# irconde/SSL4POLYP

Hardware: AMD Instinct MI355X
Metric: training-step images/sec/node, ViT-B/16 224^2 (cls fine-tune) (higher is better)
Workload: dtype bf16; 1 GPU; ViT-B/16 classification fine-tune, bs=64/GPU, 224^2, AdamW, random init, finetune mode full (finetune.py:49-91); global_batch=64, parallelism=dp1, launch=eager, lr_schedule=constant

## Files before the change

### ssl4polyp_amd/csrc/pm_attention.hip

```cpp
#include "pm_common.h"
#include <type_traits>

namespace {

template <int DH> constexpr int kTileUnroll = DH == 32 ? 2 : 1;

template <int RB> __device__ __forceinline__ int swz(int row) {
  if constexpr (RB == 64) return (row >> 2) & 3;
  else if constexpr (RB == 128) return (((row >> 1) & 1) << 2) | ((row >> 2) & 3);
  else if constexpr (RB == 384) return row & 7;
  else return row & 15;
}

constexpr int row_bytes_of(int esize, int dh) { return dh == 80 ? (esize == 2 ? 256 : 384) : dh * esize; }
template <typename T, int DH> constexpr int row_bytes() { return row_bytes_of((int)sizeof(T), DH); }

template <typename T, int DH>
__device__ __forceinline__ void load_image(char* img, const T* __restrict__ src, long ld, int rows_valid,
                                           int rows_total, int tid, int nthreads) {
  constexpr int RB = row_bytes<T, DH>();
  constexpr int CPV = DH * sizeof(T) / 16;
  constexpr int CPF = ((DH + 31) / 32) * 32 * sizeof(T) / 16;
  constexpr int EPC = 16 / sizeof(T);
  for (int id = tid; id < rows_total * CPF; id += nthreads) {
    const int row = id / CPF, c = id % CPF;
    u32x4 v = {0u, 0u, 0u, 0u};
    if (row < rows_valid && c < CPV) v = *reinterpret_cast<const u32x4*>(src + (long)row * ld + c * EPC);
    *reinterpret_cast<u32x4*>(img + row * RB + 16 * (c ^ swz<RB>(row))) = v;
  }
}

template <typename T, int DH>
__device__ __forceinline__ Frag16 frag_rows(const char* img, int rb, int kk, int lane) {
  constexpr int RB = row_bytes<T, DH>();
  const int row = rb + (lane & 31);
  const int c = 2 * kk + (lane >> 5);
  Frag16 f;
  f.u = *reinterpret_cast<const u32x4*>(img + row * RB + 16 * (c ^ swz<RB>(row)));
  return f;
}

template <typename T>
__device__ __forceinline__ Frag16 frag_global(const T* __restrict__ rowptr, bool valid, int kk, int lane) {
  constexpr int EPC = 16 / sizeof(T);
  Frag16 f;
  f.u = (u32x4){0u, 0u, 0u, 0u};
  if (valid) f.u = *reinterpret_cast<const u32x4*>(rowptr + (2 * kk + (lane >> 5)) * EPC);
  return f;
}

template <typename T, int DH>
__device__ __forceinline__ f32x16 mma_imgT_acc(const char* PM_LDS_IMAGE img, int rb, int d0, const f32x16& x, f32x16 acc, int lane) {
  constexpr int RB = row_bytes<T, DH>();
  if constexpr (sizeof(T) == 2) {
    const int g = lane >> 4, i = lane & 15, q = i >> 2, p = i & 3, hh = g >> 1;
    const int col = d0 + 16 * (g & 1) + 4 * p;
    const int c = col >> 3, sub = 8 * (p & 1);
    using lds_s4 = __attribute__((address_space(3))) short4v;
#pragma unroll
    for (int s = 0; s < 2; ++s) {
      Frag16 a, b;
      const int r0 = rb + 16 * s + 4 * hh + q;
      const int r1 = r0 + 8;
      const short4v lo = __builtin_amdgcn_ds_read_tr16_b64_v4i16((lds_s4*)(img + r0 * RB + 16 * (c ^ swz<RB>(r0)) + sub));
      const short4v hi = __builtin_amdgcn_ds_read_tr16_b64_v4i16((lds_s4*)(img + r1 * RB + 16 * (c ^ swz<RB>(r1)) + sub));
      a.u[0] = ((unsigned)(unsigned short)lo[0]) | (((unsigned)(unsigned short)lo[1]) << 16);
      a.u[1] = ((unsigned)(unsigned short)lo[2]) | (((unsigned)(unsigned short)lo[3]) << 16);
      a.u[2] = ((unsigned)(unsigned short)hi[0]) | (((unsigned)(unsigned short)hi[1]) << 16);
      a.u[3] = ((unsigned)(unsigned short)hi[2]) | (((unsigned)(unsigned short)hi[3]) << 16);
#pragma unroll
      for (int j = 0; j < 8; ++j) frag_set<T>(b, j, x[8 * s + j]);
      acc = mfma16B<T>(a, b, acc);
    }
  } else {
    const int hh = lane >> 5;
    const int col = d0 + (lane & 31);
#pragma unroll
    for (int r = 0; r < 16; ++r) {
      const int row = rb + acc_row(r, hh);
      const float a = *reinterpret_cast<const float*>(img + row * RB + 16 * ((col >> 2) ^ swz<RB>(row)) + 4 * (col & 3));
      acc = __builtin_amdgcn_mfma_f32_32x32x2f32(a, x[r], acc, 0, 0, 0);
    }
  }
  return acc;
}

__device__ __forceinline__ f32x16 zero16() {
  f32x16 z;
#pragma unroll
  for (int r = 0; r < 16; ++r) z[r] = 0.f;
  return z;
}

template <typename T>
__device__ __forceinline__ void store_tile_T(T* __restrict__ rowptr, bool valid, const f32x16& acc, float scale, int lane,
                                             int ncols = 32) {
  if (!valid) return;
  const int hh = lane >> 5;
#pragma unroll
  for (int g = 0; g < 4; ++g) {
    f32x4 v = {acc[4 * g] * scale, acc[4 * g + 1] * scale, acc[4 * g + 2] * scale, acc[4 * g + 3] * scale};
    if (8 * g + 4 * hh < ncols) store4<T>(rowptr + 8 * g + 4 * hh, v);
  }
}
template <int DH> __device__ __forceinline__ constexpr int tile_cols(int dt) { return DH - 32 * dt < 32 ? DH - 32 * dt : 32; }

constexpr float kLog2e = 1.4426950408889634f;

template <int DH> __device__ __forceinline__ int problem_of_block(int bid, int nprob, int H) {
  if constexpr (DH == 32) {
    if ((nprob & 15) == 0 && (H & 1) == 0) {
      const int xcd = bid & 7, j = bid >> 3;
      return (((j >> 1) << 3) + xcd) * 2 + (j & 1);
    }
  }
  return bid;
}

constexpr int chunk_tiles(int row_bytes, int nt) {
  const int per_tile = 2 * 32 * row_bytes + 2 * 32 * (int)sizeof(float);
  if (nt * per_tile <= 150 * 1024) return nt;
  return (80 * 1024) / per_tile;
}

template <typename T, int DH, int NT, int CT>
__global__ __launch_bounds__(NT * 64) void attn_fwd_kernel(const T* __restrict__ qkv, T* __restrict__ out,
                                                                        float* __restrict__ lse, int N, int H,
                                                                        float scale) {
  constexpr int RB = row_bytes<T, DH>();
  constexpr int KS = DH * sizeof(T) / 32;
  constexpr int DT = (DH + 31) / 32;
  extern __shared__ __attribute__((aligned(16))) char smem[];
  char* imgK = smem;
  char* imgV = smem + CT * 32 * RB;
  const int tid = threadIdx.x, lane = tid & 63, wave = tid >> 6, hh = lane >> 5;
  const int prob = problem_of_block<DH>(blockIdx.x, gridDim.x, H);
  const int b = prob / H, h = prob % H;
  const long ld = 3L * H * DH;
  const T* base = qkv + (long)b * N * ld + h * DH;
  const float c = scale * kLog2e;
  const int q = wave * 32 + (lane & 31);
  const bool qv = q < N;
  Frag16 fq[KS];
  f32x16 o[DT];
#pragma unroll
  for (int dt = 0; dt < DT; ++dt) o[dt] = zero16();
  float m = -INFINITY, l = 0.f;
  for (int c0 = 0; c0 < NT; c0 += CT) {
    if (c0) __syncthreads();
    load_image<T, DH>(imgK, base + H * DH + (long)c0 * 32 * ld, ld, N - c0 * 32, CT * 32, tid, NT * 64);
    load_image<T, DH>(imgV, base + 2 * H * DH + (long)c0 * 32 * ld, ld, N - c0 * 32, CT * 32, tid, NT * 64);
    __syncthreads();
    if (c0 == 0) {
#pragma unroll
      for (int kk = 0; kk < KS; ++kk) fq[kk] = frag_global<T>(base + (long)q * ld, qv, kk, lane);
    }
    const int cend = c0 + CT < NT ? c0 + CT : NT;
#pragma unroll 1
    for (int kt = c0; kt < cend; ++kt) {
      const int rb = (kt - c0) * 32;
      f32x16 s = zero16();
#pragma unroll
      for (int kk = 0; kk < KS; ++kk) s = mfma16B<T>(frag_rows<T, DH>(imgK, rb, kk, lane), fq[kk], s);
      float tm = -INFINITY;
      if (kt * 32 + 32 > N) {
#pragma unroll
        for (int r = 0; r < 16; ++r) {
          const int key = kt * 32 + acc_row(r, hh);
          s[r] = key < N ? s[r] : -INFINITY;
        }
      }
#pragma unroll
      for (int r = 0; r < 16; ++r) tm = fmaxf(tm, s[r]);
      tm = fmaxf(tm, __shfl_xor(tm, 32, 64));
      const float mn = fmaxf(m, tm);
      const float alpha = __builtin_amdgcn_exp2f((m - mn) * c);
      const float mnc = mn * c;
      float ts = 0.f;
#pragma unroll
      for (int r = 0; r < 16; ++r) {
        s[r] = __builtin_amdgcn_exp2f(s[r] * c - mnc);
        ts += s[r];
      }
      l = l * alpha + ts;
      const bool moved = __builtin_amdgcn_ballot_w64(mn != m) != 0;
      m = mn;
#pragma unroll
      for (int dt = 0; dt < DT; ++dt) {
        if (moved) {
#pragma unroll
          for (int r = 0; r < 16; ++r) o[dt][r] *= alpha;
        }
        o[dt] = mma_imgT_acc<T, DH>(imgV, rb, dt * 32, s, o[dt], lane);
      }
    }
  }
  l += __shfl_xor(l, 32, 64);
  if (qv && hh == 0) lse[((long)b * H + h) * N + q] = m * scale + __logf(l);
  const float inv = 1.0f / l;
  T* orow = out + ((long)b * N + q) * H * DH + h * DH;
#pragma unroll
  for (int dt = 0; dt < DT; ++dt) store_tile_T<T>(orow + dt * 32, qv, o[dt], inv, lane, tile_cols<DH>(dt));
}

template <typename T, int DH, int NT, int CT>
__global__ __launch_bounds__(NT * 64) void attn_bwd_q_kernel(const T* __restrict__ qkv, const T* __restrict__ out,
                                                                          const T* __restrict__ dout,
                                                                          const float* __restrict__ lse,
                                                                          float* __restrict__ delta, T* __restrict__ dqkv,
                                                                          int N, int H, float scale) {
  constexpr int RB = row_bytes<T, DH>();
  constexpr int KS = DH * sizeof(T) / 32;
  constexpr int DT = (DH + 31) / 32;
  constexpr int EPC = 16 / sizeof(T);
  extern __shared__ __attribute__((aligned(16))) char smem[];
  char* imgK = smem;
  char* imgV = smem + CT * 32 * RB;
  const int tid = threadIdx.x, lane = tid & 63, wave = tid >> 6, hh = lane >> 5;
  const int prob = problem_of_block<DH>(blockIdx.x, gridDim.x, H);
  const int b = prob / H, h = prob % H;
  const long ld = 3L * H * DH, ldo = (long)H * DH;
  const T* base = qkv + (long)b * N * ld + h * DH;
  const float c = scale * kLog2e;
  const int q = wave * 32 + (lane & 31);
  const bool qv = q < N;
  const long sidx = ((long)b * H + h) * N + q;
  Frag16 fq[KS], fdo[KS];
  float l2 = 0.f, dls = 0.f;
  f32x16 dq[DT];
#pragma unroll
  for (int dt = 0; dt < DT; ++dt) dq[dt] = zero16();
  for (int c0 = 0; c0 < NT; c0 += CT) {
    if (c0) __syncthreads();
    load_image<T, DH>(imgK, base + H * DH + (long)c0 * 32 * ld, ld, N - c0 * 32, CT * 32, tid, NT * 64);
    load_image<T, DH>(imgV, base + 2 * H * DH + (long)c0 * 32 * ld, ld, N - c0 * 32, CT * 32, tid, NT * 64);
    __syncthreads();
    if (c0 == 0) {
      const T* orow = out + ((long)b * N + q) * ldo + h * DH;
      const T* dorow = dout + ((long)b * N + q) * ldo + h * DH;
      float dl = 0.f;
#pragma unroll
      for (int kk = 0; kk < KS; ++kk) {
        fq[kk] = frag_global<T>(base + (long)q * ld, qv, kk, lane);
        fdo[kk] = frag_global<T>(dorow, qv, kk, lane);
        const Frag16 fo = frag_global<T>(orow, qv, kk, lane);
#pragma unroll
        for (int e = 0; e < EPC; ++e) dl += frag_get<T>(fdo[kk], e) * frag_get<T>(fo, e);
      }
      dl += __shfl_xor(dl, 32, 64);
      if (qv && hh == 0) delta[sidx] = dl;
      l2 = qv ? lse[sidx] * kLog2e : 0.f;
      dls = dl * scale;
    }
    const int cend = c0 + CT < NT ? c0 + CT : NT;
#pragma unroll kTileUnroll<DH>
    for (int kt = c0; kt < cend; ++kt) {
      const int rb = (kt - c0) * 32;
      f32x16 s = zero16(), dp = zero16();
#pragma unroll
      for (int kk = 0; kk < KS; ++kk) {
        s = mfma16B<T>(frag_rows<T, DH>(imgK, rb, kk, lane), fq[kk], s);
        dp = mfma16B<T>(frag_rows<T, DH>(imgV, rb, kk, lane), fdo[kk], dp);
      }
#pragma unroll
      for (int r = 0; r < 16; ++r) s[r] = __builtin_amdgcn_exp2f(fminf(s[r] * c - l2, 0.f)) * (dp[r] * scale - dls);
#pragma unroll
      for (int dt = 0; dt < DT; ++dt) dq[dt] = mma_imgT_acc<T, DH>(imgK, rb, dt * 32, s, dq[dt], lane);
    }
  }
  T* dqrow = dqkv + ((long)b * N + q) * ld + h * DH;
#pragma unroll
  for (int dt = 0; dt < DT; ++dt) store_tile_T<T>(dqrow + dt * 32, qv, dq[dt], 1.0f, lane, tile_cols<DH>(dt));
}

template <typename T, int DH, int NT, int CT>
__global__ __launch_bounds__(NT * 64) void attn_bwd_kv_kernel(const T* __restrict__ qkv, const T* __restrict__ dout,
                                                                           const float* __restrict__ lse,
                                                                           const float* __restrict__ delta,
                                                                           T* __restrict__ dqkv, int N, int H, float scale) {
  constexpr int RB = row_bytes<T, DH>();
  constexpr int KS = DH * sizeof(T) / 32;
  constexpr int DT = (DH + 31) / 32;
  extern __shared__ __attribute__((aligned(16))) char smem[];
  char* imgQ = smem;
  char* imgDO = smem + CT * 32 * RB;
  float* sl2 = reinterpret_cast<float*>(smem + 2 * CT * 32 * RB);
  float* sdl = sl2 + CT * 32;
  const int tid = threadIdx.x, lane = tid & 63, wave = tid >> 6, hh = lane >> 5;
  const int prob = problem_of_block<DH>(blockIdx.x, gridDim.x, H);
  const int b = prob / H, h = prob % H;
  const long ld = 3L * H * DH, ldo = (long)H * DH;
  const T* base = qkv + (long)b * N * ld + h * DH;
  const float c = scale * kLog2e;
  const int key = wave * 32 + (lane & 31);
  const bool kv = key < N;
  Frag16 fk[KS], fv[KS];
  f32x16 dk[DT], dv[DT];
#pragma unroll
  for (int dt = 0; dt < DT; ++dt) {
    dk[dt] = zero16();
    dv[dt] = zero16();
  }
  for (int c0 = 0; c0 < NT; c0 += CT) {
    if (c0) __syncthreads();
    load_image<T, DH>(imgQ, base + (long)c0 * 32 * ld, ld, N - c0 * 32, CT * 32, tid, NT * 64);
    load_image<T, DH>(imgDO, dout + ((long)b * N + c0 * 32) * ldo + h * DH, ldo, N - c0 * 32, CT * 32, tid, NT * 64);
    for (int i = tid; i < CT * 32; i += NT * 64) {
      const int qi = c0 * 32 + i;
      const long sidx = ((long)b * H + h) * N + qi;
      sl2[i] = qi < N ? lse[sidx] * kLog2e : 0.f;
      sdl[i] = qi < N ? delta[sidx] * scale : 0.f;
    }
    __syncthreads();
    if (c0 == 0) {
#pragma unroll
      for (int kk = 0; kk < KS; ++kk) {
        fk[kk] = frag_global<T>(base + (long)key * ld + H * DH, kv, kk, lane);
        fv[kk] = frag_global<T>(base + (long)key * ld + 2 * H * DH, kv, kk, lane);
      }
    }
    const int cend = c0 + CT < NT ? c0 + CT : NT;
#pragma unroll kTileUnroll<DH>
    for (int qt = c0; qt < cend; ++qt) {
      const int rb = (qt - c0) * 32;
      f32x16 s = zero16(), dp = zero16();
#pragma unroll
      for (int kk = 0; kk < KS; ++kk) {
        s = mfma16B<T>(frag_rows<T, DH>(imgQ, rb, kk, lane), fk[kk], s);
        dp = mfma16B<T>(frag_rows<T, DH>(imgDO, rb, kk, lane), fv[kk], dp);
      }
#pragma unroll
      for (int g = 0; g < 4; ++g) {
        const int qq = rb + 8 * g + 4 * hh;
        const f32x4 l4 = *reinterpret_cast<const f32x4*>(sl2 + qq);
        const f32x4 d4 = *reinterpret_cast<const f32x4*>(sdl + qq);
#pragma unroll
        for (int e = 0; e < 4; ++e) {
          const int r = 4 * g + e;
          const float p = __builtin_amdgcn_exp2f(fminf(s[r] * c - l4[e], 0.f));
          s[r] = p;
          dp[r] = p * (dp[r] * scale - d4[e]);
        }
      }
#pragma unroll
      for (int dt = 0; dt < DT; ++dt) {
        dv[dt] = mma_imgT_acc<T, DH>(imgDO, rb, dt * 32, s, dv[dt], lane);
        dk[dt] = mma_imgT_acc<T, DH>(imgQ, rb, dt * 32, dp, dk[dt], lane);
      }
    }
  }
  T* drow = dqkv + ((long)b * N + key) * ld + h * DH;
#pragma unroll
  for (int dt = 0; dt < DT; ++dt) {
    store_tile_T<T>(drow + H * DH + dt * 32, kv, dk[dt], 1.0f, lane, tile_cols<DH>(dt));
    store_tile_T<T>(drow + 2 * H * DH + dt * 32, kv, dv[dt], 1.0f, lane, tile_cols<DH>(dt));
  }
}

template <int RB, typename T> __device__ __forceinline__ void dma_rows(char* img, const T* __restrict__ base, long ld, int rows_valid,
                                                                        int piece, int lane) {
  static_assert(sizeof(T) == 2, "16-bit rows");
  constexpr int CPR = RB / 16, RPP = 1024 / RB;
  const int row = piece * RPP + lane / CPR, cs = lane % CPR;
  const int c = cs ^ swz<RB>(row);
  const int gr = row < rows_valid ? row : rows_valid - 1;
  __builtin_amdgcn_global_load_lds((const __attribute__((address_space(1))) void*)(base + (long)gr * ld + c * 8),
                                   (__attribute__((address_space(3))) void*)(img + 1024 * piece), 16, 0, 0);
}

template <typename T, int DH, int NT>
__global__ __launch_bounds__(NT * 64) void attn_fwd2_kernel(const T* __restrict__ qkv, T* __restrict__ out,
                                                           float* __restrict__ lse, int N, int H, int BH, float scale) {
  constexpr int RB = DH * 2;
  constexpr int IMG = NT * 32 * RB;
  constexpr int PCS = IMG / 1024;
  constexpr int KS = RB / 32;
  constexpr int DT = DH / 32;
  extern __shared__ __attribute__((aligned(16))) char smem[];
  char* imgQ = smem + 4 * IMG;
  const int tid = threadIdx.x, lane = tid & 63, hh = lane >> 5;
  const int wave = __builtin_amdgcn_readfirstlane(tid >> 6);
  const long hd = (long)H * DH, ld = 3 * hd;
  const float c = scale * kLog2e;
  auto issue = [&](int head, int buf) {
    const int b = head / H, h = head % H;
    const T* base = qkv + (long)b * N * ld + (long)h * DH;
    char* imgK = smem + buf * 2 * IMG;
#pragma unroll
    for (int i = 0; i < (PCS + NT - 1) / NT; ++i) {
      const int p = wave + NT * i;
      if (p < PCS) {
        dma_rows<RB>(imgK, base + hd, ld, N, p, lane);
        dma_rows<RB>(imgK + IMG, base + 2 * hd, ld, N, p, lane);
        dma_rows<RB>(imgQ, base, ld, N, p, lane);
      }
    }
  };
  int head = blockIdx.x;
  if (head >= BH) return;
  issue(head, 0);
  for (int it = 0; head < BH; head += gridDim.x, ++it) {
    const int buf = it & 1;
    const char* imgK = smem + buf * 2 * IMG;
    const char* imgV = imgK + IMG;
    asm volatile("s_waitcnt vmcnt(0)" ::: "memory");
    __syncthreads();
    Frag16 fq[KS];
#pragma unroll
    for (int kk = 0; kk < KS; ++kk) fq[kk] = frag_rows<T, DH>(imgQ, wave * 32, kk, lane);
    asm volatile("s_waitcnt lgkmcnt(0)" ::: "memory");
    __builtin_amdgcn_sched_barrier(0);
    __syncthreads();
    const int next = head + gridDim.x;
    if (next < BH) issue(next, buf ^ 1);
    const int b = head / H, h = head % H;
    f32x16 s[NT];
#pragma unroll
    for (int kt = 0; kt < NT; ++kt) {
      s[kt] = zero16();
#pragma unroll
      for (int kk = 0; kk < KS; ++kk) s[kt] = mfma16B<T>(frag_rows<T, DH>(imgK, kt * 32, kk, lane), fq[kk], s[kt]);
    }
#pragma unroll
    for (int r = 0; r < 16; ++r) {
      const int key = (NT - 1) * 32 + acc_row(r, hh);
      s[NT - 1][r] = key < N ? s[NT - 1][r] : -INFINITY;
    }
    float m = -INFINITY;
#pragma unroll
    for (int kt = 0; kt < NT; ++kt)
#pragma unroll
      for (int r = 0; r < 16; r += 2) m = fmaxf(m, fmaxf(s[kt][r], s[kt][r + 1]));
    m = fmaxf(m, __shfl_xor(m, 32, 64));
    const float mc = m * c;
    f32x16 o[DT];
#pragma unroll
    for (int dt = 0; dt < DT; ++dt) o[dt] = zero16();
    float l = 0.f;
#pragma unroll
    for (int kt = 0; kt < NT; ++kt) {
#pragma unroll
      for (int r = 0; r < 16; ++r) {
        s[kt][r] = __builtin_amdgcn_exp2f(s[kt][r] * c - mc);
        l += s[kt][r];
      }
#pragma unroll
      for (int dt = 0; dt < DT; ++dt) o[dt] = mma_imgT_acc<T, DH>(imgV, kt * 32, dt * 32, s[kt], o[dt], lane);
    }
    l += __shfl_xor(l, 32, 64);
    const int q = wave * 32 + (lane & 31);
    const bool qv = q < N;
    if (qv && hh == 0) lse[((long)b * H + h) * N + q] = m * scale + __logf(l);
    const float inv = 1.0f / l;
    T* orow = out + ((long)b * N + q) * H * DH + h * DH;
#pragma unroll
    for (int dt = 0; dt < DT; ++dt) store_tile_T<T>(orow + dt * 32, qv, o[dt], inv, lane);
  }
}

template <typename T, int DH, int NT>
__global__ __launch_bounds__(NT * 64) void attn_bwd_fused_kernel(const T* __restrict__ qkv, const T* __restrict__ out,
                                                                const T* __restrict__ dout,
                                                                const float* __restrict__ lse, T* __restrict__ dqkv,
                                                                int N, int H, float scale) {
  constexpr int RB = DH * 2;
  constexpr int IMG = NT * 32 * RB;
  constexpr int PCS = IMG / 1024;
  constexpr int KS = RB / 32;
  constexpr int DT = DH / 32;
  constexpr int CPR = RB / 16;
  extern __shared__ __attribute__((aligned(16))) char smem[];
  char* imgQ = smem;
  char* imgK = smem + IMG;
  char* imgV = smem + 2 * IMG;
  char* imgDO = smem + 3 * IMG;
  float* sl2 = reinterpret_cast<float*>(smem + 4 * IMG);
  float* sdl = sl2 + NT * 32;
  const int tid = threadIdx.x, lane = tid & 63, hh = lane >> 5;
  const int wave = __builtin_amdgcn_readfirstlane(tid >> 6);
  const int prob = problem_of_block<DH>(blockIdx.x, gridDim.x, H);
  const int b = prob / H, h = prob % H;
  const long ld = 3L * H * DH, ldo = (long)H * DH;
  const T* base = qkv + (long)b * N * ld + h * DH;
  const T* dobase = dout + (long)b * N * ldo + h * DH;
#pragma unroll
  for (int i = 0; i < (PCS + NT - 1) / NT; ++i) {
    const int p = wave + NT * i;
    if (p < PCS) {
      dma_rows<RB>(imgQ, base, ld, N, p, lane);
      dma_rows<RB>(imgK, base + H * DH, ld, N, p, lane);
      dma_rows<RB>(imgV, base + 2 * H * DH, ld, N, p, lane);
      dma_rows<RB>(imgDO, dobase, ldo, N, p, lane);
    }
  }
  const int q = wave * 32 + (lane & 31);
  const bool qv = q < N;
  const long sidx = ((long)b * H + h) * N;
  Frag16 fo[KS];
  {
    const T* orow = out + ((long)b * N + (qv ? q : N - 1)) * ldo + h * DH;
#pragma unroll
    for (int kk = 0; kk < KS; ++kk) fo[kk].u = *reinterpret_cast<const u32x4*>(orow + (2 * kk + hh) * 8);
  }
  for (int i = tid; i < NT * 32; i += NT * 64) sl2[i] = i < N ? lse[sidx + i] * kLog2e : 0.f;
  asm volatile("s_waitcnt vmcnt(0)" ::: "memory");
  __syncthreads();
  {
    const int pad0 = N, npad = NT * 32 - N;
    for (int i = tid; i < npad * CPR; i += NT * 64) {
      const int off = (pad0 + i / CPR) * RB + 16 * (i % CPR);
      const u32x4 z = {0u, 0u, 0u, 0u};
      *reinterpret_cast<u32x4*>(imgQ + off) = z;
      *reinterpret_cast<u32x4*>(imgK + off) = z;
      *reinterpret_cast<u32x4*>(imgV + off) = z;
      *reinterpret_cast<u32x4*>(imgDO + off) = z;
    }
  }
  __syncthreads();
  const float c = scale * kLog2e;
  Frag16 fq[KS], fdo[KS];
  float dl = 0.f;
#pragma unroll
  for (int kk = 0; kk < KS; ++kk) {
    fq[kk] = frag_rows<T, DH>(imgQ, wave * 32, kk, lane);
    fdo[kk] = frag_rows<T, DH>(imgDO, wave * 32, kk, lane);
#pragma unroll
    for (int e = 0; e < 8; ++e) dl += frag_get<T>(fdo[kk], e) * frag_get<T>(fo[kk], e);
  }
  dl += __shfl_xor(dl, 32, 64);
  if (!qv) dl = 0.f;
  if (hh == 0) sdl[q] = dl * scale;
  {
    const float l2 = sl2[q];
    const float dls = dl * scale;
    f32x16 dq[DT];
#pragma unroll
    for (int dt = 0; dt < DT; ++dt) dq[dt] = zero16();
#pragma unroll kTileUnroll<DH>
    for (int kt = 0; kt < NT; ++kt) {
      f32x16 s = zero16(), dp = zero16();
#pragma unroll
      for (int kk = 0; kk < KS; ++kk) {
        s = mfma16B<T>(frag_rows<T, DH>(imgK, kt * 32, kk, lane), fq[kk], s);
        dp = mfma16B<T>(frag_rows<T, DH>(imgV, kt * 32, kk, lane), fdo[kk], dp);
      }
#pragma unroll
      for (int r = 0; r < 16; ++r) s[r] = __builtin_amdgcn_exp2f(fminf(s[r] * c - l2, 0.f)) * (dp[r] * scale - dls);
#pragma unroll
      for (int dt = 0; dt < DT; ++dt) dq[dt] = mma_imgT_acc<T, DH>(imgK, kt * 32, dt * 32, s, dq[dt], lane);
    }
    T* dqrow = dqkv + ((long)b * N + q) * ld + h * DH;
#pragma unroll
    for (int dt = 0; dt < DT; ++dt) store_tile_T<T>(dqrow + dt * 32, qv, dq[dt], 1.0f, lane);
  }
  __syncthreads();
  {
    const int key = q;
    const bool kv = qv;
    Frag16 fk[KS], fv[KS];
#pragma unroll
    for (int kk = 0; kk < KS; ++kk) {
      fk[kk] = frag_rows<T, DH>(imgK, wave * 32, kk, lane);
      fv[kk] = frag_rows<T, DH>(imgV, wave * 32, kk, lane);
    }
    f32x16 dk[DT], dv[DT];
#pragma unroll
    for (int dt = 0; dt < DT; ++dt) {
      dk[dt] = zero16();
      dv[dt] = zero16();
    }
#pragma unroll kTileUnroll<DH>
    for (int qt = 0; qt < NT; ++qt) {
      f32x16 s = zero16(), dp = zero16();
#pragma unroll
      for (int kk = 0; kk < KS; ++kk) {
        s = mfma16B<T>(frag_rows<T, DH>(imgQ, qt * 32, kk, lane), fk[kk], s);
        dp = mfma16B<T>(frag_rows<T, DH>(imgDO, qt * 32, kk, lane), fv[kk], dp);
      }
#pragma unroll
      for (int g = 0; g < 4; ++g) {
        const int qq = qt * 32 + 8 * g + 4 * hh;
        const f32x4 l4 = *reinterpret_cast<const f32x4*>(sl2 + qq);
        const f32x4 d4 = *reinterpret_cast<const f32x4*>(sdl + qq);
#pragma unroll
        for (int e = 0; e < 4; ++e) {
          const int r = 4 * g + e;
          const float pr = __builtin_amdgcn_exp2f(fminf(s[r] * c - l4[e], 0.f));
          s[r] = pr;
          dp[r] = pr * (dp[r] * scale - d4[e]);
        }
      }
#pragma unroll
      for (int dt = 0; dt < DT; ++dt) {
        dv[dt] = mma_imgT_acc<T, DH>(imgDO, qt * 32, dt * 32, s, dv[dt], lane);
        dk[dt] = mma_imgT_acc<T, DH>(imgQ, qt * 32, dt * 32, dp, dk[dt], lane);
      }
    }
    T* drow = dqkv + ((long)b * N + key) * ld + h * DH;
#pragma unroll
    for (int dt = 0; dt < DT; ++dt) {
      store_tile_T<T>(drow + H * DH + dt * 32, kv, dk[dt], 1.0f, lane);
      store_tile_T<T>(drow + 2 * H * DH + dt * 32, kv, dv[dt], 1.0f, lane);
    }
  }
}

int plan_attention(bool backward, int B, int N, int H, int dh, int dtype, pm_attention_plan_info* p) {
  if (B <= 0 || N <= 0 || H <= 0) return PM_ESHAPE;
  if (N > 288) return PM_ESHAPE;
  if (dh != 32 && dh != 64 && dh != 80) return PM_ESHAPE;
  if (dtype != PM_BF16 && dtype != PM_F16 && dtype != PM_F32) return PM_EINVAL;
  const int tiles = (N + 31) / 32, BH = B * H;
  const bool half = dtype != PM_F32;
  const int rb = row_bytes_of(half ? 2 : 4, dh);
  p->nt = dh == 80 ? (tiles <= 3 ? 3 : 9) : tiles <= 1 ? 1 : tiles <= 2 ? 2 : tiles <= 7 ? 7 : 9;
  p->ct = p->nt;
  p->grid = BH;
  p->launches = 1;
  p->lds_bytes[1] = 0;
  if (!backward && half && dh == 64 && tiles == 7) {
    p->family = PM_ATTN_FWD_PERSISTENT;
    const int rounds = (BH + 255) / 256;
    p->grid = (BH + rounds - 1) / rounds;
    p->lds_bytes[0] = 5 * 7 * 32 * dh * 2;
  } else if (!backward) {
    p->family = PM_ATTN_FWD_HEAD;
    p->ct = chunk_tiles(rb, p->nt);
    p->lds_bytes[0] = 2 * p->ct * 32 * rb;
  } else if (half && dh != 80) {
    p->family = PM_ATTN_BWD_FUSED;
    p->lds_bytes[0] = 4 * p->nt * 32 * rb + 2 * p->nt * 32 * sizeof(float);
  } else {
    p->family = PM_ATTN_BWD_SPLIT;
    p->launches = 2;
    p->ct = chunk_tiles(rb, p->nt);
    p->lds_bytes[0] = 2 * p->ct * 32 * rb;
    p->lds_bytes[1] = p->lds_bytes[0] + 2 * p->ct * 32 * sizeof(float);
  }
  return PM_OK;
}

template <int N> using Tiles = std::integral_constant<int, N>;
template <int DH, typename F> int with_nt(int nt, F&& f) {
  if constexpr (DH == 80) {
    if (nt == 3) return f(Tiles<3>{});
  } else {
    if (nt == 1) return f(Tiles<1>{});
    if (nt == 2) return f(Tiles<2>{});
    if (nt == 7) return f(Tiles<7>{});
  }
  return nt == 9 ? f(Tiles<9>{}) : PM_ESHAPE;
}

template <typename T, int DH>
int launch_fwd(const pm_attention_plan_info& p, const void* qkv, void* out, float* lse, int B, int N, int H, hipStream_t s) {
  const float scale = 1.0f / sqrtf((float)DH);
  if constexpr (sizeof(T) == 2 && DH == 64) {
    if (p.family == PM_ATTN_FWD_PERSISTENT) {
      auto kern = attn_fwd2_kernel<T, 64, 7>;
      PM_ALLOW_LDS(kern, p.lds_bytes[0]);
      hipLaunchKernelGGL(kern, dim3(p.grid), dim3(7 * 64), p.lds_bytes[0], s, (const T*)qkv, (T*)out, lse, N, H, B * H, scale);
      return pm_check_launch();
    }
  }
  return with_nt<DH>(p.nt, [&](auto nt) {
    constexpr int NT = decltype(nt)::value;
    auto kern = attn_fwd_kernel<T, DH, NT, chunk_tiles(row_bytes<T, DH>(), NT)>;
    PM_ALLOW_LDS(kern, p.lds_bytes[0]);
    hipLaunchKernelGGL(kern, dim3(p.grid), dim3(NT * 64), p.lds_bytes[0], s, (const T*)qkv, (T*)out, lse, N, H, scale);
    return pm_check_launch();
  });
}

template <typename T, int DH>
int launch_bwd(const pm_attention_plan_info& p, const void* qkv, const void* out, const void* dout, const float* lse, float* delta,
               void* dqkv, int B, int N, int H, hipStream_t s) {
  const float scale = 1.0f / sqrtf((float)DH);
  return with_nt<DH>(p.nt, [&](auto nt) {
    constexpr int NT = decltype(nt)::value;
    if constexpr (sizeof(T) == 2 && DH != 80) {
      auto kern = attn_bwd_fused_kernel<T, DH, NT>;
      PM_ALLOW_LDS(kern, p.lds_bytes[0]);
      hipLaunchKernelGGL(kern, dim3(p.grid), dim3(NT * 64), p.lds_bytes[0], s, (const T*)qkv, (const T*)out, (const T*)dout, lse,
                         (T*)dqkv, N, H, scale);
    } else {
      constexpr int CT = chunk_tiles(row_bytes<T, DH>(), NT);
      auto kq = attn_bwd_q_kernel<T, DH, NT, CT>;
      auto kkv = attn_bwd_kv_kernel<T, DH, NT, CT>;
      PM_ALLOW_LDS(kq, p.lds_bytes[0]);
      PM_ALLOW_LDS(kkv, p.lds_bytes[1]);
      hipLaunchKernelGGL(kq, dim3(p.grid), dim3(NT * 64), p.lds_bytes[0], s, (const T*)qkv, (const T*)out, (const T*)dout, lse,
                         delta, (T*)dqkv, N, H, scale);
      hipLaunchKernelGGL(kkv, dim3(p.grid), dim3(NT * 64), p.lds_bytes[1], s, (const T*)qkv, (const T*)dout, lse,
                         (const float*)delta, (T*)dqkv, N, H, scale);
    }
    return pm_check_launch();
  });
}

}

extern "C" int pm_attention_plan(int backward, int B, int N, int H, int dh, int dtype, pm_attention_plan_info* info) {
  if (!info) return PM_EINVAL;
  return plan_attention(backward != 0, B, N, H, dh, dtype, info);
}

extern "C" int pm_attention_fwd(const void* qkv, void* out, float* lse, int B, int N, int H, int dh, int dtype,
                                void* stream) {
  if (!qkv || !out || !lse) return PM_EINVAL;
  pm_attention_plan_info p;
  const int st = plan_attention(false, B, N, H, dh, dtype, &p);
  if (st) return st;
  hipStream_t s = pm_stream(stream);
  PM_DISPATCH_ACT(dtype, T, {
    if (dh == 80) return launch_fwd<T, 80>(p, qkv, out, lse, B, N, H, s);
    return dh == 64 ? launch_fwd<T, 64>(p, qkv, out, lse, B, N, H, s) : launch_fwd<T, 32>(p, qkv, out, lse, B, N, H, s);
  });
}

extern "C" int pm_attention_bwd(const void* qkv, const void* out, const void* dout, const float* lse, float* delta,
                                void* dqkv, int B, int N, int H, int dh, int dtype, void* stream) {
  if (!qkv || !out || !dout || !lse || !delta || !dqkv) return PM_EINVAL;
  pm_attention_plan_info p;
  const int st = plan_attention(true, B, N, H, dh, dtype, &p);
  if (st) return st;
  hipStream_t s = pm_stream(stream);
  PM_DISPATCH_ACT(dtype, T, {
    if (dh == 80) return launch_bwd<T, 80>(p, qkv, out, dout, lse, delta, dqkv, B, N, H, s);
    return dh == 64 ? launch_bwd<T, 64>(p, qkv, out, dout, lse, delta, dqkv, B, N, H, s)
                    : launch_bwd<T, 32>(p, qkv, out, dout, lse, delta, dqkv, B, N, H, s);
  });
}
```

Before: 6251 images/sec.

## Software-pipeline attention backward tile loops in pairs with explicit MFMA/LDS scheduling

Refactors the dQ and dK/dV inner loops of the fused attention backward kernel into a shared helper that, for dh=64 and up to 8 tiles, processes tiles in pairs. The second tile's score MFMAs are issued before the first tile's softmax and product, and sched_group_barrier hints interleave LDS reads with MFMA instructions. The aim is to hide LDS latency and keep the matrix units busy. The risks are higher register pressure from holding two score tiles, and scheduling hints that may not fit the compiler's actual instruction mix.

```diff
diff --git a/ssl4polyp_amd/csrc/pm_attention.hip b/ssl4polyp_amd/csrc/pm_attention.hip
--- a/ssl4polyp_amd/csrc/pm_attention.hip
+++ b/ssl4polyp_amd/csrc/pm_attention.hip
@@ -458,6 +458,60 @@
   }
 }
 
+template <int DH, int NT> constexpr bool kTilePairs = DH == 64 && NT <= 8;
+template <int NR, int SR> __device__ __forceinline__ void sched_score_stream() {
+  __builtin_amdgcn_sched_group_barrier(0x100, 4, 0);
+#pragma unroll
+  for (int i = 0; i < NR - 4; ++i) {
+    __builtin_amdgcn_sched_group_barrier(0x008, 1, 0);
+    if (SR > 0 && i + 1 == NR / 2) __builtin_amdgcn_sched_group_barrier(0x100, SR, 0);
+    __builtin_amdgcn_sched_group_barrier(0x100, 1, 0);
+  }
+  __builtin_amdgcn_sched_group_barrier(0x008, 4, 0);
+}
+template <int PM> __device__ __forceinline__ void sched_prod_stream() {
+  __builtin_amdgcn_sched_group_barrier(0x100, 4, 0);
+#pragma unroll
+  for (int i = 0; i < PM - 2; ++i) {
+    __builtin_amdgcn_sched_group_barrier(0x008, 1, 0);
+    __builtin_amdgcn_sched_group_barrier(0x100, 2, 0);
+  }
+  __builtin_amdgcn_sched_group_barrier(0x008, 2, 0);
+}
+template <int NT, int KS, int SR, int PM, bool PAIRS, int UNROLL, typename Scores, typename Rows, typename Soft, typename Prod>
+__device__ __forceinline__ void bwd_tile_loop(Scores&& scores, Rows&& rows, Soft&& soft, Prod&& prod) {
+  constexpr int NP = PAIRS ? NT / 2 * 2 : 0;
+  constexpr int LONE_UNROLL = PAIRS ? 1 : UNROLL;
+  f32x16 s0, p0, s1, p1;
+#pragma unroll 1
+  for (int t = 0; t < NP; t += 2) {
+    scores(t, s0, p0);
+    const auto r0 = rows(t);
+    scores(t + 1, s1, p1);
+    soft(r0, s0, p0);
+    prod(t, s0, p0);
+    const auto r1 = rows(t + 1);
+    soft(r1, s1, p1);
+    prod(t + 1, s1, p1);
+    sched_score_stream<4 * KS, SR>();
+    sched_prod_stream<PM>();
+    if constexpr (SR > 0) __builtin_amdgcn_sched_group_barrier(0x100, SR, 0);
+    sched_prod_stream<PM>();
+  }
+#pragma unroll LONE_UNROLL
+  for (int t = NP; t < NT; ++t) {
+    scores(t, s0, p0);
+    const auto r0 = rows(t);
+    soft(r0, s0, p0);
+    prod(t, s0, p0);
+    if constexpr (PAIRS) {
+      sched_score_stream<2 * KS, 0>();
+      if constexpr (SR > 0) __builtin_amdgcn_sched_group_barrier(0x100, SR, 0);
+      sched_prod_stream<PM>();
+    }
+  }
+}
+
 template <typename T, int DH, int NT>
 __global__ __launch_bounds__(NT * 64) void attn_bwd_fused_kernel(const T* __restrict__ qkv, const T* __restrict__ out,
                                                                 const T* __restrict__ dout,
@@ -536,19 +590,26 @@
     f32x16 dq[DT];
 #pragma unroll
     for (int dt = 0; dt < DT; ++dt) dq[dt] = zero16();
-#pragma unroll kTileUnroll<DH>
-    for (int kt = 0; kt < NT; ++kt) {
-      f32x16 s = zero16(), dp = zero16();
-#pragma unroll
-      for (int kk = 0; kk < KS; ++kk) {
-        s = mfma16B<T>(frag_rows<T, DH>(imgK, kt * 32, kk, lane), fq[kk], s);
-        dp = mfma16B<T>(frag_rows<T, DH>(imgV, kt * 32, kk, lane), fdo[kk], dp);
-      }
-#pragma unroll
-      for (int r = 0; r < 16; ++r) s[r] = __builtin_amdgcn_exp2f(fminf(s[r] * c - l2, 0.f)) * (dp[r] * scale - dls);
-#pragma unroll
-      for (int dt = 0; dt < DT; ++dt) dq[dt] = mma_imgT_acc<T, DH>(imgK, kt * 32, dt * 32, s, dq[dt], lane);
-    }
+    struct NoRows {};
+    bwd_tile_loop<NT, KS, 0, 2 * DT, kTilePairs<DH, NT>, kTileUnroll<DH>>(
+        [&](int kt, f32x16& s, f32x16& dp) {
+          s = zero16();
+          dp = zero16();
+#pragma unroll
+          for (int kk = 0; kk < KS; ++kk) {
+            s = mfma16B<T>(frag_rows<T, DH>(imgK, kt * 32, kk, lane), fq[kk], s);
+            dp = mfma16B<T>(frag_rows<T, DH>(imgV, kt * 32, kk, lane), fdo[kk], dp);
+          }
+        },
+        [&](int) { return NoRows{}; },
+        [&](const NoRows&, f32x16& s, f32x16& dp) {
+#pragma unroll
+          for (int r = 0; r < 16; ++r) s[r] = __builtin_amdgcn_exp2f(fminf(s[r] * c - l2, 0.f)) * (dp[r] * scale - dls);
+        },
+        [&](int kt, f32x16& s, f32x16&) {
+#pragma unroll
+          for (int dt = 0; dt < DT; ++dt) dq[dt] = mma_imgT_acc<T, DH>(imgK, kt * 32, dt * 32, s, dq[dt], lane);
+        });
     T* dqrow = dqkv + ((long)b * N + q) * ld + h * DH;
 #pragma unroll
     for (int dt = 0; dt < DT; ++dt) store_tile_T<T>(dqrow + dt * 32, qv, dq[dt], 1.0f, lane);
@@ -569,33 +630,46 @@
       dk[dt] = zero16();
       dv[dt] = zero16();
     }
-#pragma unroll kTileUnroll<DH>
-    for (int qt = 0; qt < NT; ++qt) {
-      f32x16 s = zero16(), dp = zero16();
-#pragma unroll
-      for (int kk = 0; kk < KS; ++kk) {
-        s = mfma16B<T>(frag_rows<T, DH>(imgQ, qt * 32, kk, lane), fk[kk], s);
-        dp = mfma16B<T>(frag_rows<T, DH>(imgDO, qt * 32, kk, lane), fv[kk], dp);
-      }
-#pragma unroll
-      for (int g = 0; g < 4; ++g) {
-        const int qq = qt * 32 + 8 * g + 4 * hh;
-        const f32x4 l4 = *reinterpret_cast<const f32x4*>(sl2 + qq);
-        const f32x4 d4 = *reinterpret_cast<const f32x4*>(sdl + qq);
-#pragma unroll
-        for (int e = 0; e < 4; ++e) {
-          const int r = 4 * g + e;
-          const float pr = __builtin_amdgcn_exp2f(fminf(s[r] * c - l4[e], 0.f));
-          s[r] = pr;
-          dp[r] = pr * (dp[r] * scale - d4[e]);
-        }
-      }
-#pragma unroll
-      for (int dt = 0; dt < DT; ++dt) {
-        dv[dt] = mma_imgT_acc<T, DH>(imgDO, qt * 32, dt * 32, s, dv[dt], lane);
-        dk[dt] = mma_imgT_acc<T, DH>(imgQ, qt * 32, dt * 32, dp, dk[dt], lane);
-      }
-    }
+    struct TileRows { f32x4 l4[4], d4[4]; };
+    bwd_tile_loop<NT, KS, 8, 4 * DT, kTilePairs<DH, NT>, kTileUnroll<DH>>(
+        [&](int qt, f32x16& s, f32x16& dp) {
+          s = zero16();
+          dp = zero16();
+#pragma unroll
+          for (int kk = 0; kk < KS; ++kk) {
+            s = mfma16B<T>(frag_rows<T, DH>(imgQ, qt * 32, kk, lane), fk[kk], s);
+            dp = mfma16B<T>(frag_rows<T, DH>(imgDO, qt * 32, kk, lane), fv[kk], dp);
+          }
+        },
+        [&](int qt) {
+          TileRows w;
+#pragma unroll
+          for (int g = 0; g < 4; ++g) {
+            const int qq = qt * 32 + 8 * g + 4 * hh;
+            w.l4[g] = *reinterpret_cast<const f32x4*>(sl2 + qq);
+            w.d4[g] = *reinterpret_cast<const f32x4*>(sdl + qq);
+          }
+          return w;
+        },
+        [&](const TileRows& w, f32x16& s, f32x16& dp) {
+#pragma unroll
+          for (int g = 0; g < 4; ++g) {
+#pragma unroll
+            for (int e = 0; e < 4; ++e) {
+              const int r = 4 * g + e;
+              const float pr = __builtin_amdgcn_exp2f(fminf(s[r] * c - w.l4[g][e], 0.f));
+              s[r] = pr;
+              dp[r] = pr * (dp[r] * scale - w.d4[g][e]);
+            }
+          }
+        },
+        [&](int qt, f32x16& s, f32x16& dp) {
+#pragma unroll
+          for (int dt = 0; dt < DT; ++dt) {
+            dv[dt] = mma_imgT_acc<T, DH>(imgDO, qt * 32, dt * 32, s, dv[dt], lane);
+            dk[dt] = mma_imgT_acc<T, DH>(imgQ, qt * 32, dt * 32, dp, dk[dt], lane);
+          }
+        });
     T* drow = dqkv + ((long)b * N + key) * ld + h * DH;
 #pragma unroll
     for (int dt = 0; dt < DT; ++dt) {
```

Result: no change. 6256 images/sec, median of 2 (+0.1%).
